# uber-research/UPSNet

Hardware: NVIDIA H100
Metric: panoptic images/sec at 1024x2048 (higher is better)
Workload: dtype bf16x3

## Files before the change

### include/upsnet_b200.h

```cpp
#ifndef UPSNET_B200_H_
#define UPSNET_B200_H_

#include <stddef.h>
#include <stdint.h>

#ifdef __cplusplus
extern "C" {
#endif

#define UPSNET_E_BADARG (-1)
#define UPSNET_E_UNSUPPORTED (-2)
#define UPSNET_E_WORKSPACE (-3)

#define UPSNET_LAYOUT_NCHW 0
#define UPSNET_LAYOUT_NHWC 1
#define UPSNET_LAYOUT_FLAT_PAIR 2

#define UPSNET_DTYPE_F32 0
#define UPSNET_DTYPE_BF16 1
#define UPSNET_DTYPE_PAIR 2

#define UPSNET_EPI_RELU 1
#define UPSNET_EPI_RES_UP2 2
#define UPSNET_EPI_STEM_PAIR 8
// ... 31 lines not shown

int upsnet_conv2d_forward(const float *x, const float *weight, const float *bias,
                          const float *residual, float *y, int N, int Cin, int H, int W,
                          int Cout, int kh, int kw, int stride_h, int stride_w, int pad_h,
                          int pad_w, int dil_h, int dil_w, int epi_flags, int precision,
                          void *stream);

int upsnet_igemm_packed_weight_bytes(int Cout, int Cin, int kh, int kw, size_t *bytes);
int upsnet_igemm_pack_weight(const float *weight, int Cout, int Cin, int kh, int kw, void *packed,
                             void *stream);
int upsnet_igemm_forward(const void *x_nhwc, const float *offset, const float *mask,
                         const void *packed, const float *bias, const void *residual, void *y,
                         int N, int H, int W, int Cin, int Cout, int kh, int kw, int stride_h,
                         int stride_w, int pad_h, int pad_w, int dil_h, int dil_w, int out_layout,
                         int x_dtype, int y_dtype, int epi_flags, int precision, const int *n_dev, void *stream);
int upsnet_tma_set_tile_n(int bn);

int upsnet_dcn_packed_weight_bytes(int Cout, int Cin, int kh, int kw, size_t *bytes);
int upsnet_dcn_pack_weight(const float *weight, int Cout, int Cin, int kh, int kw, void *packed, void *stream);
int upsnet_dcn_pair_forward(const void *x_pair, const float *offset, const float *mask, const void *packed,
                            const float *bias, void *y_pair, int N, int H, int W, int Cin, int Cout, int kh, int kw,
                            int pad_h, int pad_w, int dil_h, int dil_w, int epi_flags, void *stream);
int upsnet_dcn_set_tile_n(int bn);

int upsnet_panoptic_workspace_bytes(int n, int H, int W, int num_thing, size_t *bytes);
int upsnet_panoptic_workspace_min_bytes(int n, int H, int W, int num_thing, size_t *bytes);
int upsnet_panoptic_head(const float *fcn, int S, int H, int W, const float *boxes,
                         const float *cls_prob, const float *mask_logit, const int64_t *cls_idx,
                         int n, const int *n_dev, int num_stuff, double fraction_threshold, int64_t *keep_out,
                         int *k_out, int64_t *labels, int64_t *sem_labels, void *workspace,
                         size_t workspace_bytes, void *stream);
int upsnet_panoptic_head_up4(const float *score, int S, int Hs, int Ws, const float *boxes,
                             const float *cls_prob, const float *mask_logit, const int64_t *cls_idx,
                             int n, const int *n_dev, int num_stuff, double fraction_threshold, int64_t *keep_out,
                             int *k_out, int64_t *labels, int64_t *sem_labels, void *workspace,
                             size_t workspace_bytes, void *stream);

int upsnet_mask_removal(const float *boxes, const float *cls_prob, const float *mask_logit,
                        const int64_t *cls_idx, int n, const int *n_dev, int H, int W, int num_thing,
                        double fraction_threshold, int64_t *keep_out, int *k_out, float *mask_energy,
                        void *workspace, size_t workspace_bytes, void *stream);

int upsnet_stem_workspace_bytes(int N, int H, int W, int kh, int kw, int pad, size_t *bytes);
int upsnet_stem_packed_weight_bytes(int Cout, int kh, size_t *bytes);
int upsnet_stem_pack_weight(const float *weight, int Cout, int Cin, int kh, int kw, void *packed,
                            void *stream);
// ... 270 lines not shown
```

### upsnet_b200/build.py

```python
import os
import shutil
import subprocess
import sys

HERE = os.path.dirname(os.path.abspath(__file__))
CSRC = os.path.join(HERE, "csrc")
LIB = os.path.join(HERE, "libupsnet_b200.so")
SOURCES = ["roi_align.cu", "nms.cu", "panoptic.cu", "igemm_simt.cu", "igemm_tc.cu", "igemm_tma.cu", "dcn_win.cu", "detection.cu", "pool.cu", "post.cu", "impost.cu", "pq.cu", "sseg.cu", "cocoeval.cu", "combined.cu", "rpn_target.cu", "proposal_target.cu", "panoptic_loss.cu", "train_loss.cu", "labels.cu", "backward.cu", "conv_backward.cu", "sgd.cu", "capi.cu"]
NVCC_FLAGS = ["-gencode", "arch=compute_90a,code=sm_90a", "-O3", "-lineinfo", "-std=c++17",
              "-Xcompiler", "-fPIC", "--expt-relaxed-constexpr"]


def nvcc():
    for home in (os.environ.get("CUDA_HOME"), os.environ.get("CUDA_PATH")):
        if home and os.path.exists(os.path.join(home, "bin", "nvcc")):
            return os.path.join(home, "bin", "nvcc")
    return shutil.which("nvcc") or "/usr/local/cuda/bin/nvcc"


def _stale():
    if not os.path.exists(LIB):
        return True
    t = os.path.getmtime(LIB)
    deps = [os.path.join(CSRC, f) for f in os.listdir(CSRC)]
    deps.append(os.path.join(HERE, "..", "include", "upsnet_b200.h"))
    return any(os.path.getmtime(d) > t for d in deps)


def build(force=False, verbose=False):
    if not force and not _stale():
        return LIB
    objs = []
    procs = []
    os.makedirs(os.path.join(HERE, "build"), exist_ok=True)
    for src in SOURCES:
        obj = os.path.join(HERE, "build", src.replace(".cu", ".o"))
        cmd = [nvcc()] + NVCC_FLAGS + (["-Xptxas", "-v"] if verbose else []) + \
              ["-c", os.path.join(CSRC, src), "-o", obj]
        procs.append((src, subprocess.Popen(cmd, stdout=subprocess.PIPE, stderr=subprocess.STDOUT, text=True)))
        objs.append(obj)
    failed = False
    for src, pr in procs:
        out, _ = pr.communicate()
        if pr.returncode != 0 or verbose:
            sys.stderr.write("== %s ==\n%s\n" % (src, out))
        failed |= pr.returncode != 0
    if failed:
        raise RuntimeError("nvcc failed")
    subprocess.check_call([nvcc()] + NVCC_FLAGS[:2] + ["-shared", "-o", LIB] + objs + ["-lcudart"])
    return LIB


if __name__ == "__main__":
    print(build(force="--force" in sys.argv, verbose="-v" in sys.argv))
```

### upsnet_b200/csrc/dcn_win.cu

```cuda
#include <cuda.h>
#include <cuda_bf16.h>

#include "common.cuh"
#include "tc_ptx.cuh"
#include "tc_params.cuh"

namespace ups {

constexpr int DW_BM = 128;
constexpr int DW_WW = 32, DW_WH = 20;
constexpr int DW_PLANE = DW_WW * DW_WH * 32;
constexpr int DW_WIN_BYTES = 2 * DW_PLANE;
constexpr int DW_WIN_BUFS = 2;
constexpr int DW_KHW = 9;
constexpr int DW_GROUPS = 2;
constexpr int DW_EPI_PITCH = 36;
constexpr uint32_t DW_EPI_BYTES = DW_BM * DW_EPI_PITCH * 4;

constexpr uint32_t DW_OFF_BARS = 0;
constexpr uint32_t DW_OFF_STATS = 192;
constexpr uint32_t DW_OFF_ORG = 256;
constexpr uint32_t DW_OFF_TW = 512;
constexpr uint32_t DW_OFF_TP = DW_OFF_TW + DW_KHW * DW_BM * 16;
constexpr uint32_t DW_OFF_STAGES = DW_OFF_TP + DW_KHW * DW_BM * 4;
static_assert(DW_OFF_STAGES % 1024 == 0, "stage buffers need 1024-byte alignment (SWIZZLE_128B)");

template <int BN> struct DwCfg {
  static constexpr int NCW = BN == 128 ? 2 : 1;
  static constexpr int FRAGS = 2 / NCW;
  static constexpr int BK = BN == 128 ? 32 : 64;
  static constexpr int SPK = BK / 16;
  static constexpr int ROWB = BK * 2;
  static constexpr int CONSUMERS = 128 * NCW;
  static constexpr int WARP_TMAB = CONSUMERS / 32, WARP_TMAW = WARP_TMAB + 1, WARP_PROD0 = WARP_TMAB + 4;
  static constexpr int GROUP = 4 * (SPK / 2) * 32;
  static constexpr int PRODUCERS = GROUP * DW_GROUPS;
  static constexpr int THREADS = WARP_PROD0 * 32 + PRODUCERS;
  static constexpr int WARPGROUPS = THREADS / 128;
  static constexpr int REGS_LAUNCH = 16384 / (32 * ((THREADS / 32 + 3) / 4)) / 8 * 8;
  static constexpr int REGS_TMA = 32, REGS_CONSUMER = 128;
  static_assert(NCW * REGS_CONSUMER + REGS_TMA + (PRODUCERS / 128) * REGS_LAUNCH <= WARPGROUPS * REGS_LAUNCH,
                "setmaxnreg budgets exceed the CTA's register allocation");
  static constexpr int TABLE_IT = (DW_KHW * DW_BM + PRODUCERS - 1) / PRODUCERS;
  static constexpr uint32_t A_BYTES = 2 * DW_BM * ROWB;
  static constexpr uint32_t B_BYTES = BN * ROWB;
  static constexpr uint32_t STAGE_BYTES = 2 * B_BYTES + A_BYTES;
  static_assert(STAGE_BYTES % 1024 == 0, "stages must keep the 1024-byte alignment of the swizzled tiles");
  static constexpr int STAGES = BN == 128 ? 3 : 2;
  static_assert(STAGES <= 3, "the barrier map holds three stages");
  static constexpr uint32_t OFF_WIN = DW_OFF_STAGES + STAGES * STAGE_BYTES;
  static constexpr uint32_t OFF_EPI = OFF_WIN + DW_WIN_BUFS * DW_WIN_BYTES;
  static constexpr uint32_t SMEM = OFF_EPI + DW_EPI_BYTES + 1024;
  static_assert(SMEM <= 227 * 1024, "shared memory exceeds 227 KB");
};
template <int ROWB> __device__ __forceinline__ uint32_t dw_chunk(uint32_t j, uint32_t r) {
  return ROWB == 128 ? (j ^ (r & 7u)) : (j ^ ((r >> 1) & 3u));
}

struct DwParams {
  const void* x;
  const float* offset;
  const float* mask;
  const float* bias;
  void* y;
  int N, H, W, Cin, Cout, Cout_pad, Ho, Wo, ph, pw, dh, dw, relu, BN, tile_w, tile_h;
};

template <int BN>
__global__ void __launch_bounds__(DwCfg<BN>::THREADS, 1)
dcn_win_kernel(const __grid_constant__ CUtensorMap tm_x, const __grid_constant__ CUtensorMap tm_w, const __grid_constant__ DwParams p) {
  using C = DwCfg<BN>;
  constexpr int DW_PRODUCERS = C::PRODUCERS, DW_CONSUMERS = C::CONSUMERS;
  constexpr int DW_WARP_TMAB = C::WARP_TMAB, DW_WARP_TMAW = C::WARP_TMAW, DW_WARP_PROD0 = C::WARP_PROD0;
  constexpr int DW_BK = C::BK, SPK = C::SPK, ROWB = C::ROWB;
  extern __shared__ __align__(1024) uint8_t smem_dyn[];
  const uint32_t raw = smem_u32(smem_dyn);
  const uint32_t base = (raw + 1023u) & ~1023u;
  uint8_t* sm = smem_dyn + (base - raw);

  const int tid = threadIdx.x, warp = tid >> 5, lane = tid & 31;
  const uint32_t b_bytes = C::B_BYTES;
  const uint32_t stage_bytes = C::STAGE_BYTES;
  constexpr uint32_t NST = C::STAGES, NWB = DW_WIN_BUFS;
  const uint32_t win_base = base + C::OFF_WIN;
  float* stf = reinterpret_cast<float*>(sm + C::OFF_EPI);
  const uint32_t bar_fa = base + DW_OFF_BARS;
  const uint32_t bar_fb = bar_fa + 24;
  const uint32_t bar_em = bar_fa + 48;
  const uint32_t bar_wf = bar_fa + 104;
  const uint32_t bar_we = bar_fa + 120;
  const uint32_t bar_og = bar_fa + 136;
  int* stats = reinterpret_cast<int*>(sm + DW_OFF_STATS);
  int4* org = reinterpret_cast<int4*>(sm + DW_OFF_ORG);
  float4* tw = reinterpret_cast<float4*>(sm + DW_OFF_TW);
// ... 9 lines not shown
  const long long num_tiles = (long long)p.N * tiles_w * tiles_h * n_tiles;

  if (warp == 0) {
    if (lane == 0) {
      for (int s = 0; s < C::STAGES; ++s) {
        mbar_init(bar_fa + 8 * s, C::GROUP / 32);
        mbar_init(bar_fb + 8 * s, 1);
        mbar_init(bar_em + 8 * s, DW_CONSUMERS / 32);
      }
      for (int s = 0; s < 2; ++s) {
        mbar_init(bar_wf + 8 * s, 1);
        mbar_init(bar_we + 8 * s, DW_PRODUCERS / 32);
        mbar_init(bar_og + 8 * s, 1);
      }
      fence_mbar_init();
      for (int i = 0; i < 2; ++i) {
        stats[i * 8 + 0] = 0x7fffffff; stats[i * 8 + 1] = 0x7fffffff;
        stats[i * 8 + 2] = -0x7fffffff; stats[i * 8 + 3] = -0x7fffffff;
        stats[i * 8 + 4] = 0; stats[i * 8 + 5] = 0; stats[i * 8 + 6] = 0; stats[i * 8 + 7] = 0;
      }
    }
    __syncwarp();
  }
  if (warp == DW_WARP_TMAB && lane == 0) prefetch_tmap(&tm_w);
  if (warp == DW_WARP_TMAW && lane == 0) prefetch_tmap(&tm_x);
  __syncthreads();

  if (warp >= DW_WARP_PROD0) {
    const int pt = tid - DW_WARP_PROD0 * 32;
    const int pw = warp - DW_WARP_PROD0;
    const int group = pw / (C::GROUP / 32);
    const int u = (pw >> 2) & (SPK / 2 - 1);
    const int quad = pw & 3;
    const int r = quad * 32 + lane;
    const __nv_bfloat16* xh = reinterpret_cast<const __nv_bfloat16*>(p.x);
    uint32_t g0 = 0, wf0 = 0;
    uint32_t wf_ready = 0;
    uint32_t tile_it = 0;
    for (long long tile = blockIdx.x; tile < num_tiles; tile += gridDim.x, ++tile_it) {
      const long long mt = tile / n_tiles;
      const int tx = (int)(mt % tiles_w), ty = (int)((mt / tiles_w) % tiles_h), n = (int)(mt / ((long long)tiles_w * tiles_h));
      const int par = (int)(tile_it & 1u);
      constexpr int TIT = C::TABLE_IT;
      float4 ewv[TIT];
      int ehl[TIT], ewl[TIT];
      bool evalid[TIT];
      int mnw = 0x7fffffff, mnh = 0x7fffffff, mxw = -0x7fffffff, mxh = -0x7fffffff, sw_ = 0, sh_ = 0, cnt = 0;
#pragma unroll
      for (int it = 0; it < TIT; ++it) {
        const int e = pt + it * DW_PRODUCERS;
        ewv[it] = make_float4(0.f, 0.f, 0.f, 0.f);
        ehl[it] = 0; ewl[it] = 0; evalid[it] = false;
        if (e < DW_KHW * DW_BM) {
          const int tap = e >> 7, rr = e & 127;
          const int ry = rr >> tw_shift;
          const int wo = tx * TW + (rr & (TW - 1)), ho = ty * TH + ry;
          if (ry < TH && wo < p.Wo && ho < p.Ho) {
            const int pp = ho * p.Wo + wo;
            const int ki = tap / 3, kj = tap - ki * 3;
            const float* offp = p.offset + ((size_t)n * 2 * DW_KHW + 2 * tap) * HoWo + pp;
            const float oh = __ldg(offp), ow = __ldg(offp + HoWo);
            const float h = (float)(ho - p.ph + ki * p.dh) + oh;
            const float w = (float)(wo - p.pw + kj * p.dw) + ow;
            if (h > -1.f && w > -1.f && h < (float)p.H && w < (float)p.W) {
              const int hl = (int)floorf(h), wl = (int)floorf(w), hh = hl + 1, wh = wl + 1;
// ... 34 lines not shown
      }
#pragma unroll
      for (int it = 0; it < TIT; ++it) {
        const int e = pt + it * DW_PRODUCERS;
        if (e < DW_KHW * DW_BM) {
          int code = 0;
          if (evalid[it]) {
            const int dx = ewl[it] - ox, dy = ehl[it] - oy;
            if (dx >= 0 && dx + 1 < DW_WW && dy >= 0 && dy + 1 < DW_WH) code = (dy * DW_WW + dx) * 32;
            else code = (int)(0x80000000u | ((uint32_t)(ehl[it] + 1) << 15) | (uint32_t)(ewl[it] + 1));
          }
          tw[e] = ewv[it];
          tp[e] = code;
        }
      }
      if (pt == 0) {
        org[par] = make_int4(ox, oy, n, 0);
        int* so = stats + (par ^ 1) * 8;
        so[0] = 0x7fffffff; so[1] = 0x7fffffff; so[2] = -0x7fffffff; so[3] = -0x7fffffff; so[4] = 0; so[5] = 0; so[6] = 0;
        mbar_arrive(bar_og + 8 * par);
      }
      named_bar<1, DW_PRODUCERS>();
      const __nv_bfloat16* ximg = xh + (size_t)n * p.H * p.W * (size_t)(2 * p.Cin);

      int rel = 0;
      for (int kb = (int)((uint32_t)(group - (int)g0) & 1u); kb < num_kb; kb += DW_GROUPS) {
        const uint32_t g = g0 + (uint32_t)kb;
        const uint32_t s = g % NST, it = g / NST;
        mbar_wait(bar_em + 8 * s, (it & 1u) ^ 1u);
        const uint32_t a_row = base + DW_OFF_STAGES + s * stage_bytes + 2 * b_bytes + (uint32_t)r * (uint32_t)ROWB;
#pragma unroll 1
        for (int pass = 0; pass < 4; ++pass) {
          const int sl = 2 * u + (pass >> 1), half = pass & 1;
          const int q = kb * SPK + sl;
          const int sc = q / DW_KHW, tap = q - sc * DW_KHW;
          const uint32_t wf = wf0 + (uint32_t)sc;
          if (wf >= wf_ready) {
            mbar_wait(bar_wf + 8 * (wf % NWB), (wf / NWB) & 1u);
            wf_ready = wf + 1;
          }
          const uint32_t wbuf = win_base + (wf % NWB) * (uint32_t)DW_WIN_BYTES;
          const int code = tp[tap * DW_BM + r];
          const uint32_t a_off = dw_chunk<ROWB>((uint32_t)(sl * 2 + half), (uint32_t)r) << 4;
          const float4 wv = tw[tap * DW_BM + r];
          uint4 hc[4], lc[4];
          if (code >= 0) {
            const uint32_t cl = (uint32_t)code, cr = cl + 32u;
            const uint32_t al = wbuf + cl + ((((cl >> 7) & 1u) ^ (uint32_t)half) << 4);
            const uint32_t ar = wbuf + cr + ((((cr >> 7) & 1u) ^ (uint32_t)half) << 4);
            hc[0] = lds128(al); hc[1] = lds128(ar); hc[2] = lds128(al + DW_WW * 32); hc[3] = lds128(ar + DW_WW * 32);
            lc[0] = lds128(al + DW_PLANE); lc[1] = lds128(ar + DW_PLANE);
            lc[2] = lds128(al + DW_PLANE + DW_WW * 32); lc[3] = lds128(ar + DW_PLANE + DW_WW * 32);
          } else {
            const int hl = (int)(((uint32_t)code >> 15) & 0xffffu) - 1, wl = (int)((uint32_t)code & 0x7fffu) - 1;
            const int h0 = max(hl, 0), h1 = min(hl + 1, p.H - 1), w0 = max(wl, 0), w1 = min(wl + 1, p.W - 1);
            const size_t pc = (size_t)(2 * p.Cin);
            const int cg = sc * 16 + half * 8;
            const __nv_bfloat16* b00 = ximg + ((size_t)h0 * p.W + w0) * pc + cg;
            const __nv_bfloat16* b01 = ximg + ((size_t)h0 * p.W + w1) * pc + cg;
            const __nv_bfloat16* b10 = ximg + ((size_t)h1 * p.W + w0) * pc + cg;
            const __nv_bfloat16* b11 = ximg + ((size_t)h1 * p.W + w1) * pc + cg;
// ... 2 lines not shown
            hc[2] = __ldg(reinterpret_cast<const uint4*>(b10)); lc[2] = __ldg(reinterpret_cast<const uint4*>(b10 + p.Cin));
            hc[3] = __ldg(reinterpret_cast<const uint4*>(b11)); lc[3] = __ldg(reinterpret_cast<const uint4*>(b11 + p.Cin));
          }
          uint4 ohi, olo;
          pair_blend8(wv, hc, lc, ohi, olo);
          sts128(a_row + a_off, ohi);
          sts128(a_row + DW_BM * ROWB + a_off, olo);
        }
        fence_proxy_async();
        __syncwarp();
        if (lane == 0) {
          mbar_arrive(bar_fa + 8 * s);
          while (rel < nsc && DW_KHW * (rel + 1) <= SPK * (kb + DW_GROUPS)) {
            mbar_arrive(bar_we + 8 * ((wf0 + (uint32_t)rel) % NWB));
            ++rel;
          }
        }
        rel = __shfl_sync(0xffffffffu, rel, 0);
      }
      if (lane == 0) {
        while (rel < nsc) { mbar_arrive(bar_we + 8 * ((wf0 + (uint32_t)rel) % NWB)); ++rel; }
      }
      __syncwarp();
      g0 += (uint32_t)num_kb;
      wf0 += (uint32_t)nsc;
    }
  } else if (warp >= DW_WARP_TMAB) {
    setmaxnreg_dec<C::REGS_TMA>();
    if (warp == DW_WARP_TMAW && lane == 0) {
      uint32_t wf = 0, ti = 0;
      for (long long tile = blockIdx.x; tile < num_tiles; tile += gridDim.x, ++ti) {
        const uint32_t par = ti & 1u;
        mbar_wait(bar_og + 8 * par, (ti >> 1) & 1u);
        const volatile int* ov = reinterpret_cast<const volatile int*>(&org[par]);
        const int4 o = make_int4(ov[0], ov[1], ov[2], 0);
        for (int f = 0; f < nsc; ++f, ++wf) {
          const uint32_t b = wf % NWB;
          mbar_wait(bar_we + 8 * b, ((wf / NWB) & 1u) ^ 1u);
          mbar_arrive_expect_tx(bar_wf + 8 * b, (uint32_t)DW_WIN_BYTES);
          const uint32_t dst = win_base + b * (uint32_t)DW_WIN_BYTES;
          tma_load_4d(dst, &tm_x, bar_wf + 8 * b, f * 16, o.x, o.y, o.z);
          tma_load_4d(dst + (uint32_t)DW_PLANE, &tm_x, bar_wf + 8 * b, p.Cin + f * 16, o.x, o.y, o.z);
        }
      }
    } else if (warp == DW_WARP_TMAB && lane == 0) {
      uint32_t g = 0;
      for (long long tile = blockIdx.x; tile < num_tiles; tile += gridDim.x) {
        const int n0 = (int)(tile % n_tiles) * BN;
        for (int kb = 0; kb < num_kb; ++kb, ++g) {
          const uint32_t s = g % NST, it = g / NST;
          mbar_wait(bar_em + 8 * s, (it & 1u) ^ 1u);
          const uint32_t stage = base + DW_OFF_STAGES + s * stage_bytes;
          mbar_arrive_expect_tx(bar_fb + 8 * s, 2 * b_bytes);
          tma_load_2d(stage, &tm_w, bar_fb + 8 * s, kb * DW_BK, n0);
          tma_load_2d(stage + b_bytes, &tm_w, bar_fb + 8 * s, kb * DW_BK, p.Cout_pad + n0);
        }
      }
    }
    __syncwarp();
  } else {
    setmaxnreg_inc<C::REGS_CONSUMER>();
    constexpr int FRAGS = C::FRAGS;
    const int wg = warp >> 2;
    const uint32_t dhi = ROWB == 128 ? wg_desc_hi(8 * ROWB) : wg_desc_hi_sw64(8 * ROWB);
    float d[FRAGS][BN / 2];
    constexpr uint32_t h16 = 64u * ROWB / 16u;
    __nv_bfloat16* yb = reinterpret_cast<__nv_bfloat16*>(p.y);
    uint32_t s = 0, ph = 0;
    for (long long tile = blockIdx.x; tile < num_tiles; tile += gridDim.x) {
      const long long mt = tile / n_tiles;
      const int n0 = (int)(tile % n_tiles) * BN;
      const int tx = (int)(mt % tiles_w), ty = (int)((mt / tiles_w) % tiles_h), n = (int)(mt / ((long long)tiles_w * tiles_h));
      int prev = -1;
      for (int kb = 0; kb < num_kb; ++kb) {
        mbar_wait(bar_fb + 8 * s, ph);
        mbar_wait(bar_fa + 8 * s, ph);
        const uint32_t st0 = base + DW_OFF_STAGES + s * stage_bytes;
        const uint32_t b_hi = wg_desc_lo(st0), b_lo = wg_desc_lo(st0 + b_bytes);
        const uint32_t a_hi = wg_desc_lo(st0 + 2 * b_bytes) + (uint32_t)(wg * FRAGS) * h16;
        const uint32_t a_lo = wg_desc_lo(st0 + 2 * b_bytes + DW_BM * ROWB) + (uint32_t)(wg * FRAGS) * h16;
        wgmma_fence();
#pragma unroll
        for (uint32_t k = 0; k < SPK; ++k) {
          const uint32_t acc = (kb | k) ? 1u : 0u;
          const uint64_t bh = wg_desc(b_hi + 2 * k, dhi), bl = wg_desc(b_lo + 2 * k, dhi);
#pragma unroll
          for (int f = 0; f < FRAGS; ++f) Wgmma<BN>::mma(d[f], wg_desc(a_lo + f * h16 + 2 * k, dhi), bh, acc);
#pragma unroll
          for (int f = 0; f < FRAGS; ++f) Wgmma<BN>::mma(d[f], wg_desc(a_hi + f * h16 + 2 * k, dhi), bl, 1u);
#pragma unroll
          for (int f = 0; f < FRAGS; ++f) Wgmma<BN>::mma(d[f], wg_desc(a_hi + f * h16 + 2 * k, dhi), bh, 1u);
        }
        wgmma_commit();
        wgmma_wait<1>();
#pragma unroll
        for (int f = 0; f < FRAGS; ++f) wgmma_fence_acc(d[f]);
        if (prev >= 0 && lane == 0) mbar_arrive(bar_em + 8 * prev);
        prev = (int)s;
        if (++s == NST) { s = 0; ph ^= 1u; }
      }
      wgmma_wait<0>();
#pragma unroll
      for (int f = 0; f < FRAGS; ++f) wgmma_fence_acc(d[f]);
      if (prev >= 0 && lane == 0) mbar_arrive(bar_em + 8 * prev);

      const int t = tid & 127;
      const int m = FRAGS == 2 ? t : 64 * wg + (t & 63);
      const int csub = FRAGS == 2 ? 0 : 16 * (t >> 6), cstep = FRAGS == 2 ? 16 : 32;
      const int ry = m >> tw_shift;
      const int wo = tx * TW + (m & (TW - 1)), ho = ty * TH + ry;
      const bool row_ok = ry < TH && wo < p.Wo && ho < p.Ho;
      __nv_bfloat16* yp = yb + (((size_t)n * p.Ho + ho) * p.Wo + wo) * (size_t)(2 * p.Cout);
      const uint32_t trow = smem_u32(stf + (size_t)m * DW_EPI_PITCH);
      for (int c32 = 0; c32 < BN; c32 += 32) {
        if (n0 + c32 >= p.Cout) break;
        named_bar(2 + wg, 128);
#pragma unroll
        for (int c = 0; c < BN; c += 32)
          if (c == c32) {
#pragma unroll
            for (int f = 0; f < FRAGS; ++f) acc_stage<BN, 32>(d[f], stf, DW_EPI_PITCH, 64 * (wg * FRAGS + f), c);
          }
        named_bar(2 + wg, 128);
        for (int cb = c32 + csub; cb < c32 + 32 && cb < BN; cb += cstep) {
          if (n0 + cb >= p.Cout) break;
          uint32_t rr[16];
          acc_ld16(trow + (uint32_t)(cb - c32) * 4u, rr);
// ... 8 lines not shown
              for (int e4 = 0; e4 < 4; ++e4) {
                const float4 bv = __ldg(reinterpret_cast<const float4*>(p.bias + co) + e4);
                o[4 * e4] += bv.x; o[4 * e4 + 1] += bv.y; o[4 * e4 + 2] += bv.z; o[4 * e4 + 3] += bv.w;
              }
            } else {
#pragma unroll
              for (int e = 0; e < 16; ++e)
                if (co + e < p.Cout) o[e] += __ldg(p.bias + co + e);
            }
          }
          if (p.relu) {
#pragma unroll
            for (int e = 0; e < 16; ++e) o[e] = fmaxf(o[e], 0.f);
          }
          uint32_t hw[8], lw[8];
#pragma unroll
          for (int e = 0; e < 8; ++e) split_pair2(o[2 * e], o[2 * e + 1], hw[e], lw[e]);
          uint4* dh_ = reinterpret_cast<uint4*>(yp + co);
          uint4* dl_ = reinterpret_cast<uint4*>(yp + p.Cout + co);
          dh_[0] = make_uint4(hw[0], hw[1], hw[2], hw[3]); dh_[1] = make_uint4(hw[4], hw[5], hw[6], hw[7]);
          dl_[0] = make_uint4(lw[0], lw[1], lw[2], lw[3]); dl_[1] = make_uint4(lw[4], lw[5], lw[6], lw[7]);
        }
      }
    }
  }
}

__global__ void dcn_win_pack_kernel(const float* __restrict__ w, int Cout, int Cin, int Cout_pad, int K,
                                    uint16_t* __restrict__ hi, uint16_t* __restrict__ lo) {
  const size_t total = (size_t)Cout_pad * K;
  for (size_t i = (size_t)blockIdx.x * blockDim.x + threadIdx.x; i < total; i += (size_t)gridDim.x * blockDim.x) {
    const int kk = (int)(i % (size_t)K), co = (int)(i / (size_t)K);
    const int sc = kk / (16 * DW_KHW), rem = kk - sc * 16 * DW_KHW, tap = rem >> 4, c = sc * 16 + (rem & 15);
    const float v = co < Cout ? w[((size_t)co * Cin + c) * DW_KHW + tap] : 0.f;
    __nv_bfloat16 h, l;
    split_bf16(v, h, l);
    hi[i] = *reinterpret_cast<const uint16_t*>(&h);
    lo[i] = *reinterpret_cast<const uint16_t*>(&l);
  }
}

static bool dw_supported(int Cin, int Cout, int kh, int kw) {
  return kh == 3 && kw == 3 && Cin % 64 == 0 && Cin >= 64 && Cout >= 1;
}

}

extern "C" int upsnet_dcn_packed_weight_bytes(int Cout, int Cin, int kh, int kw, size_t* bytes) {
  if (!bytes || Cout <= 0 || Cin <= 0) return UPSNET_E_BADARG;
  if (!ups::dw_supported(Cin, Cout, kh, kw)) return UPSNET_E_UNSUPPORTED;
  *bytes = (size_t)2 * ups::cout_pad(Cout) * (size_t)(9 * Cin) * sizeof(uint16_t);
  return 0;
}

extern "C" int upsnet_dcn_pack_weight(const float* weight, int Cout, int Cin, int kh, int kw, void* packed, void* stream) {
  if (!weight || !packed || Cout <= 0 || Cin <= 0) return UPSNET_E_BADARG;
  if (!ups::dw_supported(Cin, Cout, kh, kw)) return UPSNET_E_UNSUPPORTED;
  const int Cout_pad = ups::cout_pad(Cout), K = 9 * Cin;
  uint16_t* hi = reinterpret_cast<uint16_t*>(packed);
  uint16_t* lo = hi + (size_t)Cout_pad * K;
  const size_t total = (size_t)Cout_pad * K;
  int blocks = (int)((total + 255) / 256);
  if (blocks > ups::kNumSMs * 16) blocks = ups::kNumSMs * 16;
  ups::dcn_win_pack_kernel<<<blocks, 256, 0, (cudaStream_t)stream>>>(weight, Cout, Cin, Cout_pad, K, hi, lo);
  UPS_CHECK_LAUNCH();
  return 0;
}

static int g_dw_force_bn = 0;

extern "C" int upsnet_dcn_set_tile_n(int bn) {
  if (bn != 0 && bn != 32 && bn != 128) return UPSNET_E_BADARG;
  g_dw_force_bn = bn;
  return 0;
}

extern "C" int upsnet_dcn_pair_forward(const void* x_pair, const float* offset, const float* mask, const void* packed,
                                       const float* bias, void* y_pair, int N, int H, int W, int Cin, int Cout, int kh,
                                       int kw, int pad_h, int pad_w, int dil_h, int dil_w, int epi_flags, void* stream) {
  using namespace ups;
  if (!x_pair || !offset || !packed || !y_pair) return UPSNET_E_BADARG;
  if (N <= 0 || H <= 0 || W <= 0 || Cin <= 0 || Cout <= 0 || pad_h < 0 || pad_w < 0 || dil_h <= 0 || dil_w <= 0) return UPSNET_E_BADARG;
  if (!dw_supported(Cin, Cout, kh, kw)) return UPSNET_E_UNSUPPORTED;
  if ((Cout % 16) != 0) return UPSNET_E_UNSUPPORTED;
  if (H >= 32767 || W >= 32767) return UPSNET_E_UNSUPPORTED;
  if ((((uintptr_t)x_pair) & 15) || (((uintptr_t)packed) & 15) || (((uintptr_t)y_pair) & 15) || (bias && (((uintptr_t)bias) & 15)))
    return UPSNET_E_UNSUPPORTED;
  DwParams p{};
  p.x = x_pair; p.offset = offset; p.mask = mask; p.bias = bias; p.y = y_pair;
  p.N = N; p.H = H; p.W = W; p.Cin = Cin; p.Cout = Cout; p.Cout_pad = cout_pad(Cout);
  p.ph = pad_h; p.pw = pad_w; p.dh = dil_h; p.dw = dil_w;
  p.Ho = conv_out_size(H, pad_h, dil_h, 3, 1);
  p.Wo = conv_out_size(W, pad_w, dil_w, 3, 1);
  if (p.Ho <= 0 || p.Wo <= 0) return UPSNET_E_BADARG;
  p.relu = (epi_flags & UPSNET_EPI_RELU) ? 1 : 0;
  const int sms = num_sms();
  p.tile_w = 16; p.tile_h = 8;
  auto dtiles = [&]() { return (long long)p.N * ((p.Wo + p.tile_w - 1) / p.tile_w) * ((p.Ho + p.tile_h - 1) / p.tile_h) * (p.Cout_pad / p.BN); };
  p.BN = 128;
  const bool wide_ok = p.Cout_pad % 128 == 0;
  const bool wide = wide_ok && (g_dw_force_bn == 128 || (g_dw_force_bn == 0 && dtiles() >= sms / 4));
  if (!wide) p.BN = 32;
  if (!wide && dtiles() < sms / 2) { p.tile_w = 8; p.tile_h = 8; }
  if (!wide && dtiles() < sms / 2) { p.tile_h = 4; }
  const long long num_tiles = dtiles();
  if (num_tiles <= 0) return 0;
  const int bk = wide ? DwCfg<128>::BK : DwCfg<32>::BK;
  const size_t smem = wide ? DwCfg<128>::SMEM : DwCfg<32>::SMEM;
  EncodeTiledFn enc = tma_encoder();
  if (!enc) return UPSNET_E_UNSUPPORTED;
  CUtensorMap tm_x, tm_w;
  {
    const cuuint64_t dx[4] = {(cuuint64_t)(2 * Cin), (cuuint64_t)W, (cuuint64_t)H, (cuuint64_t)N};
    const cuuint64_t sx[3] = {(cuuint64_t)(2 * Cin) * 2, (cuuint64_t)W * (2 * Cin) * 2, (cuuint64_t)H * W * (2 * Cin) * 2};
    const cuuint32_t bx[4] = {16, DW_WW, DW_WH, 1};
    const cuuint32_t es[4] = {1, 1, 1, 1};
    if (enc(&tm_x, CU_TENSOR_MAP_DATA_TYPE_BFLOAT16, 4, const_cast<void*>(x_pair), dx, sx, bx, es, CU_TENSOR_MAP_INTERLEAVE_NONE,
            CU_TENSOR_MAP_SWIZZLE_32B, CU_TENSOR_MAP_L2_PROMOTION_L2_128B, CU_TENSOR_MAP_FLOAT_OOB_FILL_NONE) != CUDA_SUCCESS)
      return UPSNET_E_UNSUPPORTED;
    const cuuint64_t dwt[2] = {(cuuint64_t)(9 * Cin), (cuuint64_t)(2 * p.Cout_pad)};
    const cuuint64_t sw[1] = {(cuuint64_t)(9 * Cin) * 2};
    const cuuint32_t bw[2] = {(cuuint32_t)bk, (cuuint32_t)p.BN};
    if (enc(&tm_w, CU_TENSOR_MAP_DATA_TYPE_BFLOAT16, 2, const_cast<void*>(packed), dwt, sw, bw, es, CU_TENSOR_MAP_INTERLEAVE_NONE,
            bk == 64 ? CU_TENSOR_MAP_SWIZZLE_128B : CU_TENSOR_MAP_SWIZZLE_64B, CU_TENSOR_MAP_L2_PROMOTION_L2_256B,
            CU_TENSOR_MAP_FLOAT_OOB_FILL_NONE) != CUDA_SUCCESS)
      return UPSNET_E_UNSUPPORTED;
  }
  static PerDeviceOnce configured;
  if (configured.need()) {
    UPS_CUDA(cudaFuncSetAttribute(dcn_win_kernel<32>, cudaFuncAttributeMaxDynamicSharedMemorySize, 227 * 1024));
    UPS_CUDA(cudaFuncSetAttribute(dcn_win_kernel<128>, cudaFuncAttributeMaxDynamicSharedMemorySize, 227 * 1024));
  }
  dim3 grid((unsigned)(num_tiles < sms ? num_tiles : sms));
  if (wide)
    dcn_win_kernel<128><<<grid, DwCfg<128>::THREADS, smem, (cudaStream_t)stream>>>(tm_x, tm_w, p);
  else
    dcn_win_kernel<32><<<grid, DwCfg<32>::THREADS, smem, (cudaStream_t)stream>>>(tm_x, tm_w, p);
  UPS_CHECK_LAUNCH();
  return 0;
}
```

### upsnet_b200/csrc/tc_ptx.cuh

```cuda
#pragma once
#include <cuda.h>
#include <cuda_bf16.h>
#include <cstdint>
#include <cstdio>

#include "pair.cuh"

namespace ups {

__device__ __forceinline__ uint32_t smem_u32(const void* p) { return (uint32_t)__cvta_generic_to_shared(p); }

__device__ __forceinline__ void mbar_init(uint32_t bar, uint32_t count) {
  asm volatile("mbarrier.init.shared::cta.b64 [%0], %1;" ::"r"(bar), "r"(count));
}
__device__ __forceinline__ void mbar_arrive(uint32_t bar) {
  asm volatile("mbarrier.arrive.shared::cta.b64 _, [%0];" ::"r"(bar) : "memory");
}
__device__ __forceinline__ bool mbar_try_wait(uint32_t bar, uint32_t parity) {
  uint32_t ok;
  asm volatile(
      "{\n\t.reg .pred p;\n\t"
      "mbarrier.try_wait.parity.shared::cta.b64 p, [%1], %2;\n\t"
      "selp.u32 %0, 1, 0, p;\n\t}"
      : "=r"(ok) : "r"(bar), "r"(parity) : "memory");
// ... 15 lines not shown

__device__ __forceinline__ void mbar_arrive_expect_tx(uint32_t bar, uint32_t bytes) {
  asm volatile("mbarrier.arrive.expect_tx.shared::cta.b64 _, [%0], %1;" ::"r"(bar), "r"(bytes) : "memory");
}
__device__ __forceinline__ void tma_load_2d(uint32_t dst, const CUtensorMap* tm, uint32_t bar, int c0, int c1) {
  asm volatile(
      "cp.async.bulk.tensor.2d.shared::cluster.global.tile.mbarrier::complete_tx::bytes [%0], [%1, {%3, %4}], [%2];"
      ::"r"(dst), "l"(reinterpret_cast<uint64_t>(tm)), "r"(bar), "r"(c0), "r"(c1) : "memory");
}
__device__ __forceinline__ void tma_load_4d(uint32_t dst, const CUtensorMap* tm, uint32_t bar, int c0, int c1, int c2, int c3) {
  asm volatile(
      "cp.async.bulk.tensor.4d.shared::cluster.global.tile.mbarrier::complete_tx::bytes [%0], [%1, {%3, %4, %5, %6}], [%2];"
      ::"r"(dst), "l"(reinterpret_cast<uint64_t>(tm)), "r"(bar), "r"(c0), "r"(c1), "r"(c2), "r"(c3) : "memory");
}
__device__ __forceinline__ void tma_load_5d(uint32_t dst, const CUtensorMap* tm, uint32_t bar, int c0, int c1, int c2, int c3, int c4) {
  asm volatile(
      "cp.async.bulk.tensor.5d.shared::cluster.global.tile.mbarrier::complete_tx::bytes [%0], [%1, {%3, %4, %5, %6, %7}], [%2];"
      ::"r"(dst), "l"(reinterpret_cast<uint64_t>(tm)), "r"(bar), "r"(c0), "r"(c1), "r"(c2), "r"(c3), "r"(c4) : "memory");
}
__device__ __forceinline__ void tma_store_4d(const CUtensorMap* tm, uint32_t src, int c0, int c1, int c2, int c3) {
  asm volatile(
      "cp.async.bulk.tensor.4d.global.shared::cta.tile.bulk_group [%0, {%2, %3, %4, %5}], [%1];"
      ::"l"(reinterpret_cast<uint64_t>(tm)), "r"(src), "r"(c0), "r"(c1), "r"(c2), "r"(c3) : "memory");
}
__device__ __forceinline__ void bulk_commit() { asm volatile("cp.async.bulk.commit_group;" ::: "memory"); }
__device__ __forceinline__ void bulk_wait_read0() { asm volatile("cp.async.bulk.wait_group.read 0;" ::: "memory"); }
__device__ __forceinline__ void bulk_wait_read1() { asm volatile("cp.async.bulk.wait_group.read 1;" ::: "memory"); }
__device__ __forceinline__ void bulk_wait0() { asm volatile("cp.async.bulk.wait_group 0;" ::: "memory"); }
__device__ __forceinline__ void prefetch_tmap(const CUtensorMap* tm) {
  asm volatile("prefetch.tensormap [%0];" ::"l"(reinterpret_cast<uint64_t>(tm)) : "memory");
}

template <int R> __device__ __forceinline__ void setmaxnreg_inc() { asm volatile("setmaxnreg.inc.sync.aligned.u32 %0;" ::"n"(R)); }
template <int R> __device__ __forceinline__ void setmaxnreg_dec() { asm volatile("setmaxnreg.dec.sync.aligned.u32 %0;" ::"n"(R)); }

template <int N> struct Wgmma;
template <> struct Wgmma<32> {
  static __device__ __forceinline__ void mma(float (&d)[16], uint64_t da, uint64_t db, uint32_t accumulate) {
    asm volatile(
        "{\n\t.reg .pred p;\n\tsetp.ne.b32 p, %18, 0;\n\t"
        "wgmma.mma_async.sync.aligned.m64n32k16.f32.bf16.bf16 {%0, %1, %2, %3, %4, %5, %6, %7, %8, %9, %10, %11, %12, %13, %14, %15}, %16, %17, p, 1, 1, 0, 0;\n\t}"
        : "+f"(d[0]), "+f"(d[1]), "+f"(d[2]), "+f"(d[3]), "+f"(d[4]), "+f"(d[5]), "+f"(d[6]), "+f"(d[7]), "+f"(d[8]), "+f"(d[9]), "+f"(d[10]), "+f"(d[11]), "+f"(d[12]), "+f"(d[13]), "+f"(d[14]), "+f"(d[15])
        : "l"(da), "l"(db), "r"(accumulate));
  }
};
template <> struct Wgmma<64> {
// ... 128 lines not shown
```

Baseline: 128.4.

## Pre-swizzle DCN weights for bulk copies and restructure consumer/producer pipeline

Repacks the DCN weights into a pre-swizzled 32-wide K-slab image so the weight loader can use plain bulk copies instead of a 2D tensor-map TMA. It adds an optional single-consumer-warpgroup variant with more gather warps and setmaxnreg-budgeted producer registers, plus opt-in clock64 profiling counters. The consumer loop now waits for all wgmma work (wait<0>) before releasing each stage, instead of keeping one group in flight. That removes the overlap between MMA and the stage release, which may stall the producers. The default path still uses two consumer warpgroups, but it now runs the new weight layout and the changed wait.

```diff
diff --git a/include/upsnet_b200.h b/include/upsnet_b200.h
--- a/include/upsnet_b200.h
+++ b/include/upsnet_b200.h
@@ -77,6 +77,8 @@
                             const float *bias, void *y_pair, int N, int H, int W, int Cin, int Cout, int kh, int kw,
                             int pad_h, int pad_w, int dil_h, int dil_w, int epi_flags, void *stream);
 int upsnet_dcn_set_tile_n(int bn);
+int upsnet_dcn_set_wide_consumers(int warpgroups);
+int upsnet_dcn_profile_read(unsigned long long *out, int n);
 
 int upsnet_panoptic_workspace_bytes(int n, int H, int W, int num_thing, size_t *bytes);
 int upsnet_panoptic_workspace_min_bytes(int n, int H, int W, int num_thing, size_t *bytes);
diff --git a/upsnet_b200/build.py b/upsnet_b200/build.py
--- a/upsnet_b200/build.py
+++ b/upsnet_b200/build.py
@@ -27,15 +27,17 @@
     return any(os.path.getmtime(d) > t for d in deps)
 
 
-def build(force=False, verbose=False):
-    if not force and not _stale():
+def build(force=False, verbose=False, out_dir=None, defines=()):
+    lib = LIB if out_dir is None else os.path.join(out_dir, os.path.basename(LIB))
+    if out_dir is None and not force and not _stale():
         return LIB
     objs = []
     procs = []
-    os.makedirs(os.path.join(HERE, "build"), exist_ok=True)
+    obj_dir = os.path.join(HERE, "build") if out_dir is None else out_dir
+    os.makedirs(obj_dir, exist_ok=True)
     for src in SOURCES:
-        obj = os.path.join(HERE, "build", src.replace(".cu", ".o"))
-        cmd = [nvcc()] + NVCC_FLAGS + (["-Xptxas", "-v"] if verbose else []) + \
+        obj = os.path.join(obj_dir, src.replace(".cu", ".o"))
+        cmd = [nvcc()] + NVCC_FLAGS + ["-D" + d for d in defines] + (["-Xptxas", "-v"] if verbose else []) + \
               ["-c", os.path.join(CSRC, src), "-o", obj]
         procs.append((src, subprocess.Popen(cmd, stdout=subprocess.PIPE, stderr=subprocess.STDOUT, text=True)))
         objs.append(obj)
@@ -47,8 +49,8 @@
         failed |= pr.returncode != 0
     if failed:
         raise RuntimeError("nvcc failed")
-    subprocess.check_call([nvcc()] + NVCC_FLAGS[:2] + ["-shared", "-o", LIB] + objs + ["-lcudart"])
-    return LIB
+    subprocess.check_call([nvcc()] + NVCC_FLAGS[:2] + ["-shared", "-o", lib] + objs + ["-lcudart"])
+    return lib
 
 
 if __name__ == "__main__":
diff --git a/upsnet_b200/csrc/dcn_win.cu b/upsnet_b200/csrc/dcn_win.cu
--- a/upsnet_b200/csrc/dcn_win.cu
+++ b/upsnet_b200/csrc/dcn_win.cu
@@ -25,21 +25,29 @@
 constexpr uint32_t DW_OFF_STAGES = DW_OFF_TP + DW_KHW * DW_BM * 4;
 static_assert(DW_OFF_STAGES % 1024 == 0, "stage buffers need 1024-byte alignment (SWIZZLE_128B)");
 
-template <int BN> struct DwCfg {
-  static constexpr int NCW = BN == 128 ? 2 : 1;
+template <int BN, int NCW> struct DwCfg {
+  static_assert(BN == 128 || NCW == 1, "N tile 32 has one consumer warpgroup");
   static constexpr int FRAGS = 2 / NCW;
   static constexpr int BK = BN == 128 ? 32 : 64;
   static constexpr int SPK = BK / 16;
+  static constexpr int WN = BN == 128 && NCW == 1 ? 64 : BN;
   static constexpr int ROWB = BK * 2;
   static constexpr int CONSUMERS = 128 * NCW;
   static constexpr int WARP_TMAB = CONSUMERS / 32, WARP_TMAW = WARP_TMAB + 1, WARP_PROD0 = WARP_TMAB + 4;
-  static constexpr int GROUP = 4 * (SPK / 2) * 32;
+  static constexpr int PROD_WARPS = NCW == 1 ? 16 : 8;
+  static constexpr int GROUP = PROD_WARPS * 32 / DW_GROUPS;
+  static constexpr int SPLIT = GROUP / 128;
+  static constexpr int PASSES = 2 * SPK / SPLIT;
+  static_assert(SPK % SPLIT == 0, "a warp gathers whole K=16 slices");
   static constexpr int PRODUCERS = GROUP * DW_GROUPS;
   static constexpr int THREADS = WARP_PROD0 * 32 + PRODUCERS;
   static constexpr int WARPGROUPS = THREADS / 128;
   static constexpr int REGS_LAUNCH = 16384 / (32 * ((THREADS / 32 + 3) / 4)) / 8 * 8;
-  static constexpr int REGS_TMA = 32, REGS_CONSUMER = 128;
-  static_assert(NCW * REGS_CONSUMER + REGS_TMA + (PRODUCERS / 128) * REGS_LAUNCH <= WARPGROUPS * REGS_LAUNCH,
+  static constexpr int REGS_TMA = FRAGS * BN / 2 > 64 ? 24 : 32, REGS_CONSUMER = FRAGS * BN / 2 > 64 ? 168 : 128;
+  static constexpr int REGS_PRODUCER =
+      (WARPGROUPS * REGS_LAUNCH - NCW * REGS_CONSUMER - REGS_TMA) / (PRODUCERS / 128) / 8 * 8;
+  static_assert(REGS_PRODUCER <= REGS_LAUNCH && REGS_PRODUCER >= 72, "gather warps need 72 registers");
+  static_assert(NCW * REGS_CONSUMER + REGS_TMA + (PRODUCERS / 128) * REGS_PRODUCER <= WARPGROUPS * REGS_LAUNCH,
                 "setmaxnreg budgets exceed the CTA's register allocation");
   static constexpr int TABLE_IT = (DW_KHW * DW_BM + PRODUCERS - 1) / PRODUCERS;
   static constexpr uint32_t A_BYTES = 2 * DW_BM * ROWB;
@@ -53,6 +61,12 @@
   static constexpr uint32_t SMEM = OFF_EPI + DW_EPI_BYTES + 1024;
   static_assert(SMEM <= 227 * 1024, "shared memory exceeds 227 KB");
 };
+template <int BN, int WN>
+__device__ __forceinline__ void dw_mma(float (&d)[BN / 2], uint64_t a, uint32_t b, uint32_t dhi, uint32_t acc) {
+#pragma unroll
+  for (int h = 0; h < BN / WN; ++h)
+    Wgmma<WN>::mma(*reinterpret_cast<float(*)[WN / 2]>(&d[h * WN / 2]), a, wg_desc(b + (uint32_t)(h * WN * 64 / 16), dhi), acc);
+}
 template <int ROWB> __device__ __forceinline__ uint32_t dw_chunk(uint32_t j, uint32_t r) {
   return ROWB == 128 ? (j ^ (r & 7u)) : (j ^ ((r >> 1) & 3u));
 }
@@ -62,14 +76,41 @@
   const float* offset;
   const float* mask;
   const float* bias;
+  const void* w;
   void* y;
   int N, H, W, Cin, Cout, Cout_pad, Ho, Wo, ph, pw, dh, dw, relu, BN, tile_w, tile_h;
 };
 
-template <int BN>
-__global__ void __launch_bounds__(DwCfg<BN>::THREADS, 1)
-dcn_win_kernel(const __grid_constant__ CUtensorMap tm_x, const __grid_constant__ CUtensorMap tm_w, const __grid_constant__ DwParams p) {
-  using C = DwCfg<BN>;
+enum DwProf {
+  DWP_P_WIN,
+  DWP_P_EMPTY,
+  DWP_P_LOOP,
+  DWP_P_TABLE,
+  DWP_P_KB,
+  DWP_C_FULL,
+  DWP_C_LOOP,
+  DWP_C_EPI,
+  DWP_C_KB,
+  DWP_C_TILES,
+  DWP_C_WEIGHTS,
+  DWP_N
+};
+#ifdef UPSNET_DCN_PROFILE
+__device__ unsigned long long g_dw_prof[DWP_N];
+__device__ __forceinline__ void dw_prof_add(int slot, long long since) {
+  if ((threadIdx.x & 31) == 0) atomicAdd(&g_dw_prof[slot], (unsigned long long)(clock64() - since));
+}
+__device__ __forceinline__ void dw_prof_count(int slot) {
+  if ((threadIdx.x & 31) == 0) atomicAdd(&g_dw_prof[slot], 1ull);
+}
+#define DW_PROF(...) __VA_ARGS__
+#else
+#define DW_PROF(...)
+#endif
+
+template <int BN, int NCW>
+__device__ __forceinline__ void dcn_win_body(const CUtensorMap& tm_x, const DwParams& p) {
+  using C = DwCfg<BN, NCW>;
   constexpr int DW_PRODUCERS = C::PRODUCERS, DW_CONSUMERS = C::CONSUMERS;
   constexpr int DW_WARP_TMAB = C::WARP_TMAB, DW_WARP_TMAW = C::WARP_TMAW, DW_WARP_PROD0 = C::WARP_PROD0;
   constexpr int DW_BK = C::BK, SPK = C::SPK, ROWB = C::ROWB;
@@ -125,15 +166,15 @@
     }
     __syncwarp();
   }
-  if (warp == DW_WARP_TMAB && lane == 0) prefetch_tmap(&tm_w);
   if (warp == DW_WARP_TMAW && lane == 0) prefetch_tmap(&tm_x);
   __syncthreads();
 
   if (warp >= DW_WARP_PROD0) {
-    const int pt = tid - DW_WARP_PROD0 * 32;
+    if constexpr (C::REGS_PRODUCER < C::REGS_LAUNCH) setmaxnreg_dec<C::REGS_PRODUCER>();
+    const int pt0 = tid - DW_WARP_PROD0 * 32;
     const int pw = warp - DW_WARP_PROD0;
     const int group = pw / (C::GROUP / 32);
-    const int u = (pw >> 2) & (SPK / 2 - 1);
+    const int u = (pw >> 2) & (C::SPLIT - 1);
     const int quad = pw & 3;
     const int r = quad * 32 + lane;
     const __nv_bfloat16* xh = reinterpret_cast<const __nv_bfloat16*>(p.x);
@@ -144,6 +185,9 @@
       const long long mt = tile / n_tiles;
       const int tx = (int)(mt % tiles_w), ty = (int)((mt / tiles_w) % tiles_h), n = (int)(mt / ((long long)tiles_w * tiles_h));
       const int par = (int)(tile_it & 1u);
+      DW_PROF(const long long pf_t0 = clock64();)
+      int pt = pt0;
+      asm volatile("" : "+r"(pt));
       constexpr int TIT = C::TABLE_IT;
       float4 ewv[TIT];
       int ehl[TIT], ewl[TIT];
@@ -224,21 +268,26 @@
       }
       named_bar<1, DW_PRODUCERS>();
       const __nv_bfloat16* ximg = xh + (size_t)n * p.H * p.W * (size_t)(2 * p.Cin);
+      DW_PROF(dw_prof_add(DWP_P_TABLE, pf_t0); const long long pf_t1 = clock64();)
 
       int rel = 0;
       for (int kb = (int)((uint32_t)(group - (int)g0) & 1u); kb < num_kb; kb += DW_GROUPS) {
         const uint32_t g = g0 + (uint32_t)kb;
         const uint32_t s = g % NST, it = g / NST;
+        DW_PROF(dw_prof_count(DWP_P_KB); const long long pf_w = clock64();)
         mbar_wait(bar_em + 8 * s, (it & 1u) ^ 1u);
+        DW_PROF(dw_prof_add(DWP_P_EMPTY, pf_w);)
         const uint32_t a_row = base + DW_OFF_STAGES + s * stage_bytes + 2 * b_bytes + (uint32_t)r * (uint32_t)ROWB;
 #pragma unroll 1
-        for (int pass = 0; pass < 4; ++pass) {
-          const int sl = 2 * u + (pass >> 1), half = pass & 1;
+        for (int pass = 0; pass < C::PASSES; ++pass) {
+          const int sl = u * (SPK / C::SPLIT) + (pass >> 1), half = pass & 1;
           const int q = kb * SPK + sl;
           const int sc = q / DW_KHW, tap = q - sc * DW_KHW;
           const uint32_t wf = wf0 + (uint32_t)sc;
           if (wf >= wf_ready) {
+            DW_PROF(const long long pf_v = clock64();)
             mbar_wait(bar_wf + 8 * (wf % NWB), (wf / NWB) & 1u);
+            DW_PROF(dw_prof_add(DWP_P_WIN, pf_v);)
             wf_ready = wf + 1;
           }
           const uint32_t wbuf = win_base + (wf % NWB) * (uint32_t)DW_WIN_BYTES;
@@ -287,6 +336,7 @@
         while (rel < nsc) { mbar_arrive(bar_we + 8 * ((wf0 + (uint32_t)rel) % NWB)); ++rel; }
       }
       __syncwarp();
+      DW_PROF(dw_prof_add(DWP_P_LOOP, pf_t1);)
       g0 += (uint32_t)num_kb;
       wf0 += (uint32_t)nsc;
     }
@@ -310,6 +360,7 @@
       }
     } else if (warp == DW_WARP_TMAB && lane == 0) {
       uint32_t g = 0;
+      const uint8_t* wimg = reinterpret_cast<const uint8_t*>(p.w);
       for (long long tile = blockIdx.x; tile < num_tiles; tile += gridDim.x) {
         const int n0 = (int)(tile % n_tiles) * BN;
         for (int kb = 0; kb < num_kb; ++kb, ++g) {
@@ -317,8 +368,12 @@
           mbar_wait(bar_em + 8 * s, (it & 1u) ^ 1u);
           const uint32_t stage = base + DW_OFF_STAGES + s * stage_bytes;
           mbar_arrive_expect_tx(bar_fb + 8 * s, 2 * b_bytes);
-          tma_load_2d(stage, &tm_w, bar_fb + 8 * s, kb * DW_BK, n0);
-          tma_load_2d(stage + b_bytes, &tm_w, bar_fb + 8 * s, kb * DW_BK, p.Cout_pad + n0);
+#pragma unroll
+          for (int pl = 0; pl < 2; ++pl)
+#pragma unroll
+            for (int h = 0; h < DW_BK / 32; ++h)
+              bulk_load(stage + pl * b_bytes + h * (uint32_t)(BN * 64),
+                        wimg + ((size_t)((kb * (DW_BK / 32) + h) * 2 + pl) * p.Cout_pad + n0) * 64, BN * 64, bar_fb + 8 * s);
         }
       }
     }
@@ -328,6 +383,8 @@
     constexpr int FRAGS = C::FRAGS;
     const int wg = warp >> 2;
     const uint32_t dhi = ROWB == 128 ? wg_desc_hi(8 * ROWB) : wg_desc_hi_sw64(8 * ROWB);
+    const uint32_t dhb = wg_desc_hi_sw64(8 * 64);
+    constexpr uint32_t bslab = BN * 64 / 16;
     float d[FRAGS][BN / 2];
     constexpr uint32_t h16 = 64u * ROWB / 16u;
     __nv_bfloat16* yb = reinterpret_cast<__nv_bfloat16*>(p.y);
@@ -336,10 +393,13 @@
       const long long mt = tile / n_tiles;
       const int n0 = (int)(tile % n_tiles) * BN;
       const int tx = (int)(mt % tiles_w), ty = (int)((mt / tiles_w) % tiles_h), n = (int)(mt / ((long long)tiles_w * tiles_h));
-      int prev = -1;
+      DW_PROF(dw_prof_count(DWP_C_TILES); const long long cf_t0 = clock64();)
       for (int kb = 0; kb < num_kb; ++kb) {
+        DW_PROF(dw_prof_count(DWP_C_KB); const long long cf_w = clock64();)
         mbar_wait(bar_fb + 8 * s, ph);
+        DW_PROF(dw_prof_add(DWP_C_WEIGHTS, cf_w);)
         mbar_wait(bar_fa + 8 * s, ph);
+        DW_PROF(dw_prof_add(DWP_C_FULL, cf_w);)
         const uint32_t st0 = base + DW_OFF_STAGES + s * stage_bytes;
         const uint32_t b_hi = wg_desc_lo(st0), b_lo = wg_desc_lo(st0 + b_bytes);
         const uint32_t a_hi = wg_desc_lo(st0 + 2 * b_bytes) + (uint32_t)(wg * FRAGS) * h16;
@@ -348,26 +408,24 @@
 #pragma unroll
         for (uint32_t k = 0; k < SPK; ++k) {
           const uint32_t acc = (kb | k) ? 1u : 0u;
-          const uint64_t bh = wg_desc(b_hi + 2 * k, dhi), bl = wg_desc(b_lo + 2 * k, dhi);
-#pragma unroll
-          for (int f = 0; f < FRAGS; ++f) Wgmma<BN>::mma(d[f], wg_desc(a_lo + f * h16 + 2 * k, dhi), bh, acc);
-#pragma unroll
-          for (int f = 0; f < FRAGS; ++f) Wgmma<BN>::mma(d[f], wg_desc(a_hi + f * h16 + 2 * k, dhi), bl, 1u);
-#pragma unroll
-          for (int f = 0; f < FRAGS; ++f) Wgmma<BN>::mma(d[f], wg_desc(a_hi + f * h16 + 2 * k, dhi), bh, 1u);
+#pragma unroll
+          for (int f = 0; f < FRAGS; ++f)
+            dw_mma<BN, C::WN>(d[f], wg_desc(a_lo + f * h16 + 2 * k, dhi), b_hi + (k >> 1) * bslab + 2 * (k & 1), dhb, acc);
+#pragma unroll
+          for (int f = 0; f < FRAGS; ++f)
+            dw_mma<BN, C::WN>(d[f], wg_desc(a_hi + f * h16 + 2 * k, dhi), b_lo + (k >> 1) * bslab + 2 * (k & 1), dhb, 1u);
+#pragma unroll
+          for (int f = 0; f < FRAGS; ++f)
+            dw_mma<BN, C::WN>(d[f], wg_desc(a_hi + f * h16 + 2 * k, dhi), b_hi + (k >> 1) * bslab + 2 * (k & 1), dhb, 1u);
         }
         wgmma_commit();
-        wgmma_wait<1>();
+        wgmma_wait<0>();
 #pragma unroll
         for (int f = 0; f < FRAGS; ++f) wgmma_fence_acc(d[f]);
-        if (prev >= 0 && lane == 0) mbar_arrive(bar_em + 8 * prev);
-        prev = (int)s;
+        if (lane == 0) mbar_arrive(bar_em + 8 * s);
         if (++s == NST) { s = 0; ph ^= 1u; }
       }
-      wgmma_wait<0>();
-#pragma unroll
-      for (int f = 0; f < FRAGS; ++f) wgmma_fence_acc(d[f]);
-      if (prev >= 0 && lane == 0) mbar_arrive(bar_em + 8 * prev);
+      DW_PROF(dw_prof_add(DWP_C_LOOP, cf_t0); const long long cf_t1 = clock64();)
 
       const int t = tid & 127;
       const int m = FRAGS == 2 ? t : 64 * wg + (t & 63);
@@ -422,12 +480,23 @@
           dl_[0] = make_uint4(lw[0], lw[1], lw[2], lw[3]); dl_[1] = make_uint4(lw[4], lw[5], lw[6], lw[7]);
         }
       }
+      DW_PROF(dw_prof_add(DWP_C_EPI, cf_t1);)
     }
   }
 }
 
+template <int BN>
+__global__ void __launch_bounds__(DwCfg<BN, BN == 128 ? 2 : 1>::THREADS, 1)
+dcn_win_kernel(const __grid_constant__ CUtensorMap tm_x, const __grid_constant__ DwParams p) {
+  dcn_win_body<BN, BN == 128 ? 2 : 1>(tm_x, p);
+}
+__global__ void __launch_bounds__(DwCfg<128, 1>::THREADS, 1)
+dcn_win_1wg_kernel(const __grid_constant__ CUtensorMap tm_x, const __grid_constant__ DwParams p) {
+  dcn_win_body<128, 1>(tm_x, p);
+}
+
 __global__ void dcn_win_pack_kernel(const float* __restrict__ w, int Cout, int Cin, int Cout_pad, int K,
-                                    uint16_t* __restrict__ hi, uint16_t* __restrict__ lo) {
+                                    uint16_t* __restrict__ img) {
   const size_t total = (size_t)Cout_pad * K;
   for (size_t i = (size_t)blockIdx.x * blockDim.x + threadIdx.x; i < total; i += (size_t)gridDim.x * blockDim.x) {
     const int kk = (int)(i % (size_t)K), co = (int)(i / (size_t)K);
@@ -435,8 +504,11 @@
     const float v = co < Cout ? w[((size_t)co * Cin + c) * DW_KHW + tap] : 0.f;
     __nv_bfloat16 h, l;
     split_bf16(v, h, l);
-    hi[i] = *reinterpret_cast<const uint16_t*>(&h);
-    lo[i] = *reinterpret_cast<const uint16_t*>(&l);
+    const int slab = kk >> 5, j = (kk >> 3) & 3;
+    const size_t row = (size_t)slab * 2 * Cout_pad + co;
+    const size_t o = row * 32 + (size_t)((j ^ ((co >> 1) & 3)) * 8 + (kk & 7));
+    img[o] = *reinterpret_cast<const uint16_t*>(&h);
+    img[o + (size_t)Cout_pad * 32] = *reinterpret_cast<const uint16_t*>(&l);
   }
 }
 
@@ -457,22 +529,41 @@
   if (!weight || !packed || Cout <= 0 || Cin <= 0) return UPSNET_E_BADARG;
   if (!ups::dw_supported(Cin, Cout, kh, kw)) return UPSNET_E_UNSUPPORTED;
   const int Cout_pad = ups::cout_pad(Cout), K = 9 * Cin;
-  uint16_t* hi = reinterpret_cast<uint16_t*>(packed);
-  uint16_t* lo = hi + (size_t)Cout_pad * K;
   const size_t total = (size_t)Cout_pad * K;
   int blocks = (int)((total + 255) / 256);
   if (blocks > ups::kNumSMs * 16) blocks = ups::kNumSMs * 16;
-  ups::dcn_win_pack_kernel<<<blocks, 256, 0, (cudaStream_t)stream>>>(weight, Cout, Cin, Cout_pad, K, hi, lo);
+  ups::dcn_win_pack_kernel<<<blocks, 256, 0, (cudaStream_t)stream>>>(weight, Cout, Cin, Cout_pad, K, reinterpret_cast<uint16_t*>(packed));
   UPS_CHECK_LAUNCH();
   return 0;
 }
 
 static int g_dw_force_bn = 0;
+static int g_dw_wide_cwg = 2;
 
 extern "C" int upsnet_dcn_set_tile_n(int bn) {
   if (bn != 0 && bn != 32 && bn != 128) return UPSNET_E_BADARG;
   g_dw_force_bn = bn;
   return 0;
+}
+
+extern "C" int upsnet_dcn_set_wide_consumers(int warpgroups) {
+  if (warpgroups != 1 && warpgroups != 2) return UPSNET_E_BADARG;
+  g_dw_wide_cwg = warpgroups;
+  return 0;
+}
+
+extern "C" int upsnet_dcn_profile_read(unsigned long long* out, int n) {
+#ifdef UPSNET_DCN_PROFILE
+  if (!out || n != ups::DWP_N) return UPSNET_E_BADARG;
+  UPS_CUDA(cudaDeviceSynchronize());
+  UPS_CUDA(cudaMemcpyFromSymbol(out, ups::g_dw_prof, sizeof(unsigned long long) * ups::DWP_N));
+  const unsigned long long zero[ups::DWP_N] = {};
+  UPS_CUDA(cudaMemcpyToSymbol(ups::g_dw_prof, zero, sizeof(zero)));
+  return 0;
+#else
+  (void)out; (void)n;
+  return UPSNET_E_UNSUPPORTED;
+#endif
 }
 
 extern "C" int upsnet_dcn_pair_forward(const void* x_pair, const float* offset, const float* mask, const void* packed,
@@ -487,7 +578,7 @@
   if ((((uintptr_t)x_pair) & 15) || (((uintptr_t)packed) & 15) || (((uintptr_t)y_pair) & 15) || (bias && (((uintptr_t)bias) & 15)))
     return UPSNET_E_UNSUPPORTED;
   DwParams p{};
-  p.x = x_pair; p.offset = offset; p.mask = mask; p.bias = bias; p.y = y_pair;
+  p.x = x_pair; p.w = packed; p.offset = offset; p.mask = mask; p.bias = bias; p.y = y_pair;
   p.N = N; p.H = H; p.W = W; p.Cin = Cin; p.Cout = Cout; p.Cout_pad = cout_pad(Cout);
   p.ph = pad_h; p.pw = pad_w; p.dh = dil_h; p.dw = dil_w;
   p.Ho = conv_out_size(H, pad_h, dil_h, 3, 1);
@@ -505,11 +596,10 @@
   if (!wide && dtiles() < sms / 2) { p.tile_h = 4; }
   const long long num_tiles = dtiles();
   if (num_tiles <= 0) return 0;
-  const int bk = wide ? DwCfg<128>::BK : DwCfg<32>::BK;
-  const size_t smem = wide ? DwCfg<128>::SMEM : DwCfg<32>::SMEM;
+  const size_t smem = !wide ? DwCfg<32, 1>::SMEM : g_dw_wide_cwg == 1 ? DwCfg<128, 1>::SMEM : DwCfg<128, 2>::SMEM;
   EncodeTiledFn enc = tma_encoder();
   if (!enc) return UPSNET_E_UNSUPPORTED;
-  CUtensorMap tm_x, tm_w;
+  CUtensorMap tm_x;
   {
     const cuuint64_t dx[4] = {(cuuint64_t)(2 * Cin), (cuuint64_t)W, (cuuint64_t)H, (cuuint64_t)N};
     const cuuint64_t sx[3] = {(cuuint64_t)(2 * Cin) * 2, (cuuint64_t)W * (2 * Cin) * 2, (cuuint64_t)H * W * (2 * Cin) * 2};
@@ -518,24 +608,20 @@
     if (enc(&tm_x, CU_TENSOR_MAP_DATA_TYPE_BFLOAT16, 4, const_cast<void*>(x_pair), dx, sx, bx, es, CU_TENSOR_MAP_INTERLEAVE_NONE,
             CU_TENSOR_MAP_SWIZZLE_32B, CU_TENSOR_MAP_L2_PROMOTION_L2_128B, CU_TENSOR_MAP_FLOAT_OOB_FILL_NONE) != CUDA_SUCCESS)
       return UPSNET_E_UNSUPPORTED;
-    const cuuint64_t dwt[2] = {(cuuint64_t)(9 * Cin), (cuuint64_t)(2 * p.Cout_pad)};
-    const cuuint64_t sw[1] = {(cuuint64_t)(9 * Cin) * 2};
-    const cuuint32_t bw[2] = {(cuuint32_t)bk, (cuuint32_t)p.BN};
-    if (enc(&tm_w, CU_TENSOR_MAP_DATA_TYPE_BFLOAT16, 2, const_cast<void*>(packed), dwt, sw, bw, es, CU_TENSOR_MAP_INTERLEAVE_NONE,
-            bk == 64 ? CU_TENSOR_MAP_SWIZZLE_128B : CU_TENSOR_MAP_SWIZZLE_64B, CU_TENSOR_MAP_L2_PROMOTION_L2_256B,
-            CU_TENSOR_MAP_FLOAT_OOB_FILL_NONE) != CUDA_SUCCESS)
-      return UPSNET_E_UNSUPPORTED;
   }
   static PerDeviceOnce configured;
   if (configured.need()) {
     UPS_CUDA(cudaFuncSetAttribute(dcn_win_kernel<32>, cudaFuncAttributeMaxDynamicSharedMemorySize, 227 * 1024));
     UPS_CUDA(cudaFuncSetAttribute(dcn_win_kernel<128>, cudaFuncAttributeMaxDynamicSharedMemorySize, 227 * 1024));
+    UPS_CUDA(cudaFuncSetAttribute(dcn_win_1wg_kernel, cudaFuncAttributeMaxDynamicSharedMemorySize, 227 * 1024));
   }
   dim3 grid((unsigned)(num_tiles < sms ? num_tiles : sms));
-  if (wide)
-    dcn_win_kernel<128><<<grid, DwCfg<128>::THREADS, smem, (cudaStream_t)stream>>>(tm_x, tm_w, p);
+  if (!wide)
+    dcn_win_kernel<32><<<grid, DwCfg<32, 1>::THREADS, smem, (cudaStream_t)stream>>>(tm_x, p);
+  else if (g_dw_wide_cwg == 1)
+    dcn_win_1wg_kernel<<<grid, DwCfg<128, 1>::THREADS, smem, (cudaStream_t)stream>>>(tm_x, p);
   else
-    dcn_win_kernel<32><<<grid, DwCfg<32>::THREADS, smem, (cudaStream_t)stream>>>(tm_x, tm_w, p);
+    dcn_win_kernel<128><<<grid, DwCfg<128, 2>::THREADS, smem, (cudaStream_t)stream>>>(tm_x, p);
   UPS_CHECK_LAUNCH();
   return 0;
 }
diff --git a/upsnet_b200/csrc/tc_ptx.cuh b/upsnet_b200/csrc/tc_ptx.cuh
--- a/upsnet_b200/csrc/tc_ptx.cuh
+++ b/upsnet_b200/csrc/tc_ptx.cuh
@@ -61,6 +61,10 @@
   asm volatile(
       "cp.async.bulk.tensor.4d.global.shared::cta.tile.bulk_group [%0, {%2, %3, %4, %5}], [%1];"
       ::"l"(reinterpret_cast<uint64_t>(tm)), "r"(src), "r"(c0), "r"(c1), "r"(c2), "r"(c3) : "memory");
+}
+__device__ __forceinline__ void bulk_load(uint32_t dst_smem, const void* src, uint32_t bytes, uint32_t bar) {
+  asm volatile("cp.async.bulk.shared::cluster.global.mbarrier::complete_tx::bytes [%0], [%1], %2, [%3];"
+               :: "r"(dst_smem), "l"(src), "r"(bytes), "r"(bar) : "memory");
 }
 __device__ __forceinline__ void bulk_commit() { asm volatile("cp.async.bulk.commit_group;" ::: "memory"); }
 __device__ __forceinline__ void bulk_wait_read0() { asm volatile("cp.async.bulk.wait_group.read 0;" ::: "memory"); }
```

Result: no change. 128.8 (median of 6 runs) (+0.3%).
